# jmhb0/view_neti

Measured on AMD Instinct MI355X. Metric: TI train steps/sec (SD-1.5 512^2 bs=4 per GPU), higher is better.
Workload: dtype f16; 1 GPU; learnable_mode 0, sd15 shapes, 512x512 fp16, bs=4/GPU, grad_accum 1, full train step (VAE+16xCLIP+UNet fwd/bwd+AdamW); global_batch=4, parallelism=dp1, rccl_ranks=1, hipgraph=True

## Files before the change

### include/vneti.h

```cpp
#ifndef VNETI_H
#define VNETI_H
#include <stddef.h>
#include <stdint.h>

#ifdef __cplusplus
extern "C" {
#endif

#define VNETI_ABI_VERSION 1

int vneti_version(void);
int vneti_precision(void);
int vneti_last_error(char* buf, size_t n);

typedef struct vneti_gemm_desc {
  const void* A;
  const void* B;
  void* C;
  long long lda, ldb, ldc;
  int M, N, K;
  int batch;
  long long strideA, strideB, strideC;
  const float* bias;
  const void* rowadd;
// ... 83 lines not shown
int vneti_attn_bwd_delta(const void* dO, long long lddo, const void* O, long long ldo,
                         float* delta, int Bn, int H, int Nq, int D, void* stream);
int vneti_attn_bwd_dq(const void* Q, long long ldq, const void* K, long long ldk, const void* V,
                      long long ldv, const void* dO, long long lddo, const float* lse, float* delta,
                      const void* O, long long ldo, void* dQ, long long lddq, int Bn, int H, int Nq,
                      int Nk, int D, float scale, int causal, void* stream);
int vneti_attn_bwd_dkv(const void* Q, long long ldq, const void* K, long long ldk, const void* V,
                       long long ldv, const void* dO, long long lddo, const float* lse,
                       const float* delta, void* dK, long long lddk, void* dV, long long lddv,
                       int Bn, int H, int Nq, int Nk, int D, float scale, int causal, float* ws,
                       long long ws_floats, void* stream);
int vneti_attn_bwd_small(const void* Q, long long ldq, const void* K, long long ldk, const void* V, long long ldv,
                         const void* dO, long long lddo, const void* O, long long ldo, const float* lse, void* dQ,
                         long long lddq, void* dK, long long lddk, void* dV, long long lddv, int Bn, int H, int N, int D,
                         float scale, int causal, void* stream);
int vneti_softmax_rows_f16(void* x, long long ld, int rows, int cols, void* stream);

int vneti_add_f16(const void* a, long long lda, const void* b, long long ldb, void* out,
                  long long ldo, int rows, int cols, void* stream);
int vneti_geglu_fwd(const void* p, long long ldp, void* out, long long ldo, int rows, int C4,
                    void* stream);
int vneti_geglu_bwd(const void* dy, long long lddy, const void* p, long long ldp, void* dp,
                    long long lddp, int rows, int C4, void* stream);
int vneti_act_fwd_f16(const void* x, void* y, long long n, int act, void* stream);
int vneti_act_bwd_f16(const void* dy, const void* x, void* dx, long long n, int act, void* stream);
int vneti_timestep_embedding(const void* t, void* out, int Bn, int dim, void* stream);
int vneti_sum2x2_f16(const void* in, long long ldi, void* out, long long ldo, int Bn, int H, int W,
                     int C, void* stream);
int vneti_rng_fill_normal(void* out_f32, long long n, const void* state, unsigned stream_id,
                          void* stream);
// ... 74 lines not shown
                                  const int* slot, long long slot_stride, int accumulate, int nl, int Bn, int enc_dim,
                                  int pe_dim, void* stream);
int vneti_text_embed(const float* tok_emb, const float* pos_emb, const void* ids_i64,
                     const int* pos_obj, const float* word_obj, const int* pos_view,
                     const float* word_view, float* X, int nl, int Bn, int L, int D, void* stream);
int vneti_text_final_fwd(const float* last, const float* gamma, const float* beta, float eps,
                         const int* pos_obj, const float* bypass_obj, float alpha_obj,
                         int unconstrained_obj, const int* pos_view, const float* bypass_view,
                         float alpha_view, int unconstrained_view, float* norm_terms, void* ctx_k,
                         void* ctx_v, int nl, int Bn, int L, int D, void* stream);
int vneti_text_final_bwd(const float* last, const float* gamma, float eps, const int* pos_obj,
                         const float* bypass_obj, float alpha_obj, int unconstrained_obj,
                         float* dbypass_obj, const int* pos_view, const float* bypass_view,
                         float alpha_view, int unconstrained_view, float* dbypass_view,
                         const float* norm_terms, const void* dctx_k, const void* dctx_v, float* dX,
                         int nl, int Bn, int L, int D, void* stream);
int vneti_mapper_inputs(const void* timesteps_i64, const float* view_params, int nv, float* data,
                        int nl, int Bn, void* stream);
int vneti_cast_f32_f16(const float* x, void* y, long long n, void* stream);


int vneti_img_resample_ksize(int in_size, int out_size, int filter);
int vneti_img_resample_coeffs(int in_size, int out_size, int filter, int* bounds, int* kk, void* stream);
int vneti_img_resample_pass(const void* in, int in_w, void* out, int out_h, int out_w, const int* bounds,
                            const int* kk, int ksize, int horizontal, void* stream);
int vneti_img_crop(const void* in, int in_w, int top, int left, void* out, int h, int w, int flip, void* stream);
int vneti_img_enhance(void* img, int h, int w, int mode, float alpha, void* scratch8, void* stream);
int vneti_img_hue(void* img, int h, int w, int shift, void* stream);
int vneti_img_blur5(const void* in, void* out, float* tmp, int h, int w, const float* k5_host, void* stream);
int vneti_img_affine_nearest(const void* in, void* out, int h, int w, const int* a6_host, int fill, void* stream);
int vneti_img_to_f32_chw(const void* img, float* out, int h, int w, void* stream);
// ... 23 lines not shown
```

### view_neti_amd/csrc/attention.hip

```cpp
#include "common.h"
#include "../../include/vneti.h"

namespace {

constexpr float LOG2E = 1.4426950408889634f;
constexpr int TROW64 = 144;
constexpr int TROW32 = 80;
constexpr int DKV_QH(int D) { return D <= 64 ? 2 : 1; }

template <int D>
struct Cfg {
  static constexpr int KS = (D + 15) / 16;
  static constexpr int DPAD = KS * 16;
  static constexpr int DB = (D + 31) / 32;
  static constexpr int DCH = D / 8;
  static constexpr int ROW = DPAD * 2 + 16;
};

struct AttnArgs {
  const half_t *Q, *K, *V, *dO;
  half_t *O, *dQ, *dK, *dV;
  float* lse;
  const float* lse_in;
  const float* delta;
// ... 633 lines not shown
      for (int qd = 0; qd < 4; ++qd) {
        int d = db * 32 + 8 * qd + 4 * h2;
        if (d < D) {
          half4 k4 = {(half_t)(dk[db][4 * qd] * a.scale), (half_t)(dk[db][4 * qd + 1] * a.scale),
                      (half_t)(dk[db][4 * qd + 2] * a.scale), (half_t)(dk[db][4 * qd + 3] * a.scale)};
          half4 v4 = {(half_t)dv[db][4 * qd], (half_t)dv[db][4 * qd + 1], (half_t)dv[db][4 * qd + 2],
                      (half_t)dv[db][4 * qd + 3]};
          *reinterpret_cast<half4*>(krow + d) = k4;
          *reinterpret_cast<half4*>(vrow + d) = v4;
        }
      }
    }
  }
}

template <int D>
__global__ __launch_bounds__(256, 2) void attn_bwd_small_kernel(AttnArgs a) {
  using C = Cfg<D>;
  constexpr int NR = 96;
  constexpr int TILE = NR * C::ROW + 128;
  __shared__ __attribute__((aligned(16))) char smem[4 * TILE + 2 * NR * 4];
  char* Qs = smem;
  char* Ks = smem + TILE;
  char* Vs = smem + 2 * TILE;
  char* dOs = smem + 3 * TILE;
  float* lses = reinterpret_cast<float*>(smem + 4 * TILE);
  float* dels = lses + NR;

  const int tid = threadIdx.x, lane = tid & 63, wave = tid >> 6;
  const int l31 = lane & 31, h2 = lane >> 5;
  const int b = blockIdx.y, h = blockIdx.x;
  const int N = a.Nq;

  __amdgpu_buffer_rsrc_t rsQ = vn_make_rsrc(a.Q, (uint32_t)((long long)a.Bn * N * a.ldq * 2));
  __amdgpu_buffer_rsrc_t rsdO = vn_make_rsrc(a.dO, (uint32_t)((long long)a.Bn * N * a.lddo * 2));
// ... 4 lines not shown
  constexpr int NIT = (NR * C::DCH + 255) / 256;
  u32x4 rq[NIT], rk[NIT], rv[NIT], rd[NIT];
#pragma unroll
  for (int i = 0; i < NIT; ++i) {
    const int idx = tid + 256 * i;
    const int r = idx / C::DCH, cc = idx - r * C::DCH;
    const bool ok = idx < NR * C::DCH && r < N;
    const long long row = (long long)b * N + r;
    rq[i] = vn_buf_load16(rsQ, ok ? (uint32_t)((row * a.ldq + h * D + cc * 8) * 2) : VN_OOB);
    rk[i] = vn_buf_load16(rsK, ok ? (uint32_t)((row * a.ldk + h * D + cc * 8) * 2) : VN_OOB);
    rv[i] = vn_buf_load16(rsV, ok ? (uint32_t)((row * a.ldv + h * D + cc * 8) * 2) : VN_OOB);
    rd[i] = vn_buf_load16(rsdO, ok ? (uint32_t)((row * a.lddo + h * D + cc * 8) * 2) : VN_OOB);
  }
  float lreg = INFINITY;
  if (tid < NR && tid < N) lreg = a.lse_in[((long long)b * a.H + h) * N + tid] * LOG2E;
  zero_lds(smem, 4 * TILE);
  __syncthreads();
#pragma unroll
  for (int i = 0; i < NIT; ++i) {
    const int idx = tid + 256 * i;
    const int r = idx / C::DCH, cc = idx - r * C::DCH;
    if (idx < NR * C::DCH) {
      *reinterpret_cast<u32x4*>(Qs + r * C::ROW + cc * 16) = rq[i];
      *reinterpret_cast<u32x4*>(Ks + r * C::ROW + cc * 16) = rk[i];
      *reinterpret_cast<u32x4*>(Vs + r * C::ROW + cc * 16) = rv[i];
      *reinterpret_cast<u32x4*>(dOs + r * C::ROW + cc * 16) = rd[i];
    }
  }
  if (tid < NR) lses[tid] = lreg;
  __syncthreads();

  const float c = a.scale * LOG2E;
  const int row = wave * 32 + l31;
  const bool rok = row < N;
  if (wave < 3) {
    half8 qf[C::KS], dof[C::KS];
    float part = 0.f;
#pragma unroll
    for (int ks = 0; ks < C::KS; ++ks) {
      const int ch = ks * 2 + h2;
      qf[ks] = as_half8(*reinterpret_cast<const u32x4*>(Qs + row * C::ROW + ch * 16));
      dof[ks] = as_half8(*reinterpret_cast<const u32x4*>(dOs + row * C::ROW + ch * 16));
      const uint32_t offo = (rok && ch < C::DCH) ? (uint32_t)((((long long)b * N + row) * a.ldo + h * D + ch * 8) * 2) : VN_OOB;
      const half8 of = as_half8(vn_buf_load16(rsO, offo));
#pragma unroll
      for (int j = 0; j < 8; ++j) part += (float)dof[ks][j] * (float)of[j];
    }
    const float dlt = part + __shfl_xor(part, 32, 64);
    if (h2 == 0) dels[row] = dlt;
    const float lse2 = lses[row];
    f32x16 dq[C::DB];
#pragma unroll
    for (int i = 0; i < C::DB; ++i)
#pragma unroll
      for (int e = 0; e < 16; ++e) dq[i][e] = 0.f;
    const int nkb = a.causal ? wave + 1 : 3;
    for (int aa = 0; aa < nkb; ++aa) {
      f32x16 s, dp;
#pragma unroll
      for (int e = 0; e < 16; ++e) {
        s[e] = 0.f;
        dp[e] = 0.f;
      }
#pragma unroll
      for (int ks = 0; ks < C::KS; ++ks) {
        const int off = (aa * 32 + l31) * C::ROW + (ks * 2 + h2) * 16;
        half8 kf = as_half8(*reinterpret_cast<const u32x4*>(Ks + off));
        half8 vf = as_half8(*reinterpret_cast<const u32x4*>(Vs + off));
        s = VN_MFMA_32x32x16(kf, qf[ks], s, 0, 0, 0);
        dp = VN_MFMA_32x32x16(vf, dof[ks], dp, 0, 0, 0);
      }
      if (aa * 32 + 32 > N || (a.causal && aa == wave)) {
#pragma unroll
        for (int r = 0; r < 16; ++r) {
          const int key = aa * 32 + (r & 3) + 8 * (r >> 2) + 4 * h2;
          const bool ok = key < N && (!a.causal || key <= row);
          if (!ok) s[r] = -INFINITY;
        }
      }
#pragma unroll
      for (int r = 0; r < 16; r += 2) {
        const f32x2 t = pk_fma(f32x2{s[r], s[r + 1]}, f32x2{c, c}, f32x2{-lse2, -lse2});
        const f32x2 g = f32x2{dp[r], dp[r + 1]} - f32x2{dlt, dlt};
        const f32x2 ds = f32x2{fast_exp2(t.x), fast_exp2(t.y)} * g;
        s[r] = ds.x;
        s[r + 1] = ds.y;
      }
#pragma unroll
      for (int j = 0; j < 2; ++j) {
        half8 pf = cvt8(s, j);
#pragma unroll
        for (int db = 0; db < C::DB; ++db) {
          half8 tf = load_tr(Ks, C::ROW, db * 32, aa * 32 + 16 * j + 4 * h2, lane);
          dq[db] = VN_MFMA_32x32x16(tf, pf, dq[db], 0, 0, 0);
        }
      }
    }
    if (rok) {
      half_t* orow = a.dQ + ((long long)b * N + row) * a.lddq + h * D;
#pragma unroll
      for (int db = 0; db < C::DB; ++db)
#pragma unroll
        for (int qd = 0; qd < 4; ++qd) {
          const int d = db * 32 + 8 * qd + 4 * h2;
          if (d < D) {
            half4 v = {(half_t)(dq[db][4 * qd] * a.scale), (half_t)(dq[db][4 * qd + 1] * a.scale),
                       (half_t)(dq[db][4 * qd + 2] * a.scale), (half_t)(dq[db][4 * qd + 3] * a.scale)};
            *reinterpret_cast<half4*>(orow + d) = v;
          }
        }
    }
  }
  __syncthreads();
  if (wave < 3) {
    half8 kf[C::KS], vf[C::KS];
#pragma unroll
    for (int ks = 0; ks < C::KS; ++ks) {
      const int ch = ks * 2 + h2;
      kf[ks] = as_half8(*reinterpret_cast<const u32x4*>(Ks + row * C::ROW + ch * 16));
      vf[ks] = as_half8(*reinterpret_cast<const u32x4*>(Vs + row * C::ROW + ch * 16));
    }
    f32x16 dk[C::DB], dv[C::DB];
#pragma unroll
    for (int i = 0; i < C::DB; ++i)
#pragma unroll
      for (int e = 0; e < 16; ++e) {
        dk[i][e] = 0.f;
        dv[i][e] = 0.f;
      }
    for (int hq = a.causal ? wave : 0; hq < 3; ++hq) {
      f32x16 s, dp;
#pragma unroll
      for (int e = 0; e < 16; ++e) {
        s[e] = 0.f;
        dp[e] = 0.f;
      }
#pragma unroll
      for (int ks = 0; ks < C::KS; ++ks) {
        const int off = (hq * 32 + l31) * C::ROW + (ks * 2 + h2) * 16;
        half8 qfr = as_half8(*reinterpret_cast<const u32x4*>(Qs + off));
        half8 dofr = as_half8(*reinterpret_cast<const u32x4*>(dOs + off));
        s = VN_MFMA_32x32x16(qfr, kf[ks], s, 0, 0, 0);
        dp = VN_MFMA_32x32x16(dofr, vf[ks], dp, 0, 0, 0);
      }
#pragma unroll
      for (int qd = 0; qd < 4; ++qd) {
        f32x4 l4 = *reinterpret_cast<const f32x4*>(&lses[hq * 32 + 8 * qd + 4 * h2]);
        f32x4 d4 = *reinterpret_cast<const f32x4*>(&dels[hq * 32 + 8 * qd + 4 * h2]);
#pragma unroll
        for (int e = 0; e < 4; e += 2) {
          const int r = 4 * qd + e;
          const f32x2 t = pk_fma(f32x2{s[r], s[r + 1]}, f32x2{c, c}, -f32x2{l4[e], l4[e + 1]});
          f32x2 p = f32x2{fast_exp2(t.x), fast_exp2(t.y)};
          if (a.causal) {
// ... 2 lines not shown
            if (row > qq + 1) p.y = 0.f;
          }
          const f32x2 ds = p * (f32x2{dp[r], dp[r + 1]} - f32x2{d4[e], d4[e + 1]});
          s[r] = p.x;
          s[r + 1] = p.y;
          dp[r] = ds.x;
          dp[r + 1] = ds.y;
        }
      }
#pragma unroll
      for (int j = 0; j < 2; ++j) {
        half8 pf = cvt8(s, j);
        half8 dsf = cvt8(dp, j);
#pragma unroll
        for (int db = 0; db < C::DB; ++db) {
          half8 dot = load_tr(dOs, C::ROW, db * 32, hq * 32 + 16 * j + 4 * h2, lane);
          half8 qtf = load_tr(Qs, C::ROW, db * 32, hq * 32 + 16 * j + 4 * h2, lane);
          dv[db] = VN_MFMA_32x32x16(dot, pf, dv[db], 0, 0, 0);
          dk[db] = VN_MFMA_32x32x16(qtf, dsf, dk[db], 0, 0, 0);
        }
      }
    }
    if (rok) {
      half_t* krow = a.dK + ((long long)b * N + row) * a.lddk + h * D;
      half_t* vrow = a.dV + ((long long)b * N + row) * a.lddv + h * D;
#pragma unroll
      for (int db = 0; db < C::DB; ++db)
#pragma unroll
        for (int qd = 0; qd < 4; ++qd) {
          const int d = db * 32 + 8 * qd + 4 * h2;
          if (d < D) {
            half4 k4 = {(half_t)(dk[db][4 * qd] * a.scale), (half_t)(dk[db][4 * qd + 1] * a.scale),
                        (half_t)(dk[db][4 * qd + 2] * a.scale), (half_t)(dk[db][4 * qd + 3] * a.scale)};
            half4 v4 = {(half_t)dv[db][4 * qd], (half_t)dv[db][4 * qd + 1], (half_t)dv[db][4 * qd + 2],
                        (half_t)dv[db][4 * qd + 3]};
            *reinterpret_cast<half4*>(krow + d) = k4;
            *reinterpret_cast<half4*>(vrow + d) = v4;
          }
        }
    }
  }
}

__global__ __launch_bounds__(256) void attn_dkv_reduce_kernel(AttnArgs a) {
  const int Cc = a.H * a.D;
  const long long rows = (long long)a.Bn * a.Nk;
  const long long plane = rows * Cc;
  const unsigned gid = blockIdx.x * 256u + threadIdx.x;
  if (gid >= (unsigned)(plane / 4)) return;
  const unsigned e32 = gid * 4u;
  const unsigned row32 = e32 / (unsigned)Cc;
  const int c = (int)(e32 - row32 * (unsigned)Cc);
  const long long e = e32, row = row32;
  f32x4 k = {0.f, 0.f, 0.f, 0.f}, v = {0.f, 0.f, 0.f, 0.f};
  for (int s = 0; s < a.qsplit; ++s) {
// ... 156 lines not shown
    if (qsplit < 2) qsplit = 1;
  }
  a.qsplit = qsplit;
  a.ws = ws;
  dim3 grid(nkb * qsplit, H, Bn);
  hipStream_t st = (hipStream_t)stream;
  DISPATCH_D(attn_dkv_kernel, grid, st, a);
  if (qsplit > 1) {
    long long n4 = (long long)Bn * Nk * H * D / 4;
    VN_REQUIRE(n4 * 4 < 0x7fffffffLL, "attn_bwd_dkv: q-split reduce indexes with 32 bits");
    hipLaunchKernelGGL(attn_dkv_reduce_kernel, dim3((unsigned)cdivl(n4, 256)), dim3(256), 0, st, a);
  }
  return vneti_check_launch("attn_bwd_dkv");
}

extern "C" int vneti_attn_bwd_small(const void* Q, long long ldq, const void* K, long long ldk, const void* V, long long ldv,
                                    const void* dO, long long lddo, const void* O, long long ldo, const float* lse, void* dQ,
                                    long long lddq, void* dK, long long lddk, void* dV, long long lddv, int Bn, int H, int N,
                                    int D, float scale, int causal, void* stream) {
  VN_REQUIRE(Q && K && V && dO && O && lse && dQ && dK && dV, "attn_bwd_small: null pointer");
  VN_REQUIRE(Bn > 0 && H > 0 && N > 0, "attn_bwd_small: bad shape B=%d H=%d N=%d", Bn, H, N);
  if (N > 96 || D != 64) return VNETI_EUNSUP;
  VN_REQUIRE(ldq % 8 == 0 && ldk % 8 == 0 && ldv % 8 == 0 && lddo % 8 == 0 && ldo % 8 == 0 && lddq % 4 == 0 && lddk % 4 == 0 &&
                 lddv % 4 == 0, "attn_bwd_small: bad strides");
  AttnArgs a;
  memset(&a, 0, sizeof(a));
  a.Q = (const half_t*)Q;
  a.K = (const half_t*)K;
  a.V = (const half_t*)V;
  a.dO = (const half_t*)dO;
// ... 24 lines not shown
```

### view_neti_amd/csrc/text.hip

```cpp
#include "common.h"
#include "../../include/vneti.h"

namespace {

constexpr int MAXH = 192;

struct MapperParams {
  int w0, b0, g1, be1, w3, b3, g2, be2, wo, bo;
  int E, hd, OD, D;
};

__device__ __forceinline__ float leaky(float x) { return x > 0.f ? x : 0.01f * x; }

constexpr int MT = 1024;

__device__ __forceinline__ float group16_sum(float s) {
  s += vn_row_ror<8>(s);
  s += vn_row_ror<4>(s);
  s += vn_row_ror<2>(s);
  s += vn_row_ror<1>(s);
  return s;
}

__device__ __forceinline__ float block_sum(float v, float* red) {
// ... 631 lines not shown
#pragma unroll
          for (int j = 0; j < 8; ++j) x[i][j] += f * bv[i][j];
      }
      changed = true;
    }
  }
  if (changed) row_stats(x, D, eps, mean, rstd);
  row_ln_store(x, D, lane, mean, rstd, gamma, beta, ctx_v + row * D);
}

__global__ __launch_bounds__(256) void text_final_bwd_kernel(const float* __restrict__ last,
                                                             const float* __restrict__ gamma, float eps,
                                                             BypassArgs obj, BypassArgs view,
                                                             const half_t* __restrict__ dctx_k,
                                                             const half_t* __restrict__ dctx_v,
                                                             float* __restrict__ dX, int nl, int Bn, int L, int D) {
  const long long row = (long long)blockIdx.x * 4 + (threadIdx.x >> 6);
  const int lane = threadIdx.x & 63;
  if (row >= (long long)nl * Bn * L) return;
  const int pos = (int)(row % L);
  const int b = (int)((row / L) % Bn);
  const int l = (int)(row / ((long long)L * Bn));
  float x[TMAX][8], g1[TMAX][8];
  row_load(last + row * D, D, lane, x);
  row_ln_bwd(x, dctx_k + row * D, D, lane, eps, gamma, g1);
  const bool is_obj = obj.pos && obj.pos[b] == pos;
  const bool is_view = view.pos && view.pos[b] == pos;
  float g2[TMAX][8];
  if (!is_obj && !is_view) {
    row_ln_bwd(x, dctx_v + row * D, D, lane, eps, gamma, g2);
  } else {
// ... 17 lines not shown
#pragma unroll
      for (int j = 0; j < 8; ++j) {
        g2[i][j] = unc ? 0.f : g[i][j] + a.alpha * ug * x[i][j] / nx;
        if (c * 8 < D) dbp[c * 8 + j] = f * (g[i][j] - bv[i][j] / nb * ug);
      }
    }
  }
#pragma unroll
  for (int i = 0; i < TMAX; ++i) {
    int c = lane + 64 * i;
    if (c * 8 < D) {
      f32x4 o0 = {g1[i][0] + g2[i][0], g1[i][1] + g2[i][1], g1[i][2] + g2[i][2], g1[i][3] + g2[i][3]};
      f32x4 o1 = {g1[i][4] + g2[i][4], g1[i][5] + g2[i][5], g1[i][6] + g2[i][6], g1[i][7] + g2[i][7]};
      *reinterpret_cast<f32x4*>(dX + row * D + c * 8) = o0;
      *reinterpret_cast<f32x4*>(dX + row * D + c * 8 + 4) = o1;
    }
  }
}

__global__ void mapper_inputs_kernel(const long long* __restrict__ t, const float* __restrict__ view_params, int nv,
                                     float* __restrict__ data, int nl, int Bn) {
  int gid = blockIdx.x * blockDim.x + threadIdx.x;
  int nf = 2 + nv;
  if (gid >= nl * Bn * nf) return;
  int f = gid % nf;
  int r = gid / nf;
  int b = r % Bn, l = r / Bn;
  float v;
  if (f == 0) v = (float)t[b] / 1000.f * 2.f - 1.f;
  else if (f == 1) v = (float)l / (float)nl * 2.f - 1.f;
// ... 185 lines not shown
               uv ? norm_terms + (long long)nl * Bn : nullptr};
  if (uo || uv)
    hipLaunchKernelGGL(text_norm_terms_kernel, dim3(nl * Bn), dim3(256), 0, ST, last, o, uo ? 1 : 0, norm_terms, nl,
                       Bn, L, D);
  long long rows = (long long)nl * Bn * L;
  hipLaunchKernelGGL(text_final_fwd_kernel, dim3((unsigned)cdivl(rows, 4)), dim3(256), 0, ST, last, gamma, beta, eps, o,
                     v, (half_t*)ctx_k, (half_t*)ctx_v, nl, Bn, L, D);
  return vneti_check_launch("text_final_fwd");
}

extern "C" int vneti_text_final_bwd(const float* last, const float* gamma, float eps, const int* pos_obj,
                                    const float* bypass_obj, float alpha_obj, int unconstrained_obj,
                                    float* dbypass_obj, const int* pos_view, const float* bypass_view,
                                    float alpha_view, int unconstrained_view, float* dbypass_view,
                                    const float* norm_terms, const void* dctx_k, const void* dctx_v, float* dX,
                                    int nl, int Bn, int L, int D, void* stream) {
  VN_REQUIRE(last && gamma && dctx_k && dctx_v && dX && D % 8 == 0 && D <= 8 * 64 * TMAX, "text_final_bwd: bad arguments");
  VN_REQUIRE(!(pos_obj && bypass_obj && !dbypass_obj) && !(pos_view && bypass_view && !dbypass_view),
             "text_final_bwd: missing bypass gradient buffer");
  const bool uo = unconstrained_obj && pos_obj && bypass_obj, uv = unconstrained_view && pos_view && bypass_view;
  VN_REQUIRE(!(uo || uv) || norm_terms, "text_final_bwd: unconstrained bypass needs the forward's norm_terms");
  BypassArgs o{pos_obj && bypass_obj ? pos_obj : nullptr, bypass_obj, dbypass_obj, alpha_obj, uo ? norm_terms : nullptr};
  BypassArgs v{pos_view && bypass_view ? pos_view : nullptr, bypass_view, dbypass_view, alpha_view,
               uv ? norm_terms + (long long)nl * Bn : nullptr};
  long long rows = (long long)nl * Bn * L;
  hipLaunchKernelGGL(text_final_bwd_kernel, dim3((unsigned)cdivl(rows, 4)), dim3(256), 0, ST, last, gamma, eps, o, v,
                     (const half_t*)dctx_k, (const half_t*)dctx_v, dX, nl, Bn, L, D);
  return vneti_check_launch("text_final_bwd");
}

extern "C" int vneti_mapper_inputs(const void* timesteps, const float* view_params, int nv, float* data, int nl,
                                   int Bn, void* stream) {
  VN_REQUIRE(timesteps && data && nl > 0 && Bn > 0 && nv >= 0 && (nv == 0 || view_params), "mapper_inputs: bad arguments");
  int n = nl * Bn * (2 + nv);
  hipLaunchKernelGGL(mapper_inputs_kernel, dim3(cdiv(n, 256)), dim3(256), 0, ST, (const long long*)timesteps,
                     view_params, nv, data, nl, Bn);
  return vneti_check_launch("mapper_inputs");
}

extern "C" int vneti_cast_f32_f16(const float* x, void* y, long long n, void* stream) {
  VN_REQUIRE(x && y && n > 0 && n % 8 == 0, "cast_f32_f16: n must be a positive multiple of 8");
  hipLaunchKernelGGL(cast_f32_f16_kernel, dim3((unsigned)cdivl(n / 8, 256)), dim3(256), 0, ST, x, (half_t*)y, n / 8);
// ... 3 lines not shown
```

### view_neti_amd/engine/text.py

```python
from __future__ import annotations

from functools import partial
from typing import Dict, Optional

import torch

from .. import ops
from .. import sd_config as sc
from .schedule import Schedule, rup


class MapperState:

    def __init__(self, params: torch.Tensor, w_enc: Optional[torch.Tensor], norm_scale: Optional[float], alpha: float,
                 hidden: int = 64, enc_dim: int = 64, unconstrained: bool = False, nested_dropout_prob: float = 0.0,
                 slot: Optional[torch.Tensor] = None, slot_stride: int = 0, legacy_w_pe: Optional[torch.Tensor] = None,
                 output_bypass: bool = True, slots: Optional[torch.Tensor] = None):
        self.output_bypass = output_bypass
        self.legacy_w_pe = legacy_w_pe
        self.pe_dim = 2 * legacy_w_pe.shape[0] if legacy_w_pe is not None else 0
        self.params = params
        self.w_enc = w_enc
        self.norm_scale = norm_scale
        self.alpha = alpha
# ... 208 lines not shown
        act = ops.ACT_QUICK_GELU if cfg.act == "quick_gelu" else ops.ACT_GELU
        for i in range(cfg.num_layers):
            p = f"text_model.encoder.layers.{i}."
            r = dict(x_in=x, act=act)
            n1, r["ln1"] = self._ln(x, p + "layer_norm1", w)
            wqkv = torch.cat([w[p + "self_attn.q_proj.weight"], w[p + "self_attn.k_proj.weight"],
                              w[p + "self_attn.v_proj.weight"]], 0)
            bqkv = torch.cat([w[p + "self_attn.q_proj.bias"], w[p + "self_attn.k_proj.bias"],
                              w[p + "self_attn.v_proj.bias"]], 0)
            r["wqkv"], r_bqkv = self._w16(wqkv), self._w32(bqkv)
            qkv = self._buf((Rt, 3 * D))
            f.append(partial(ops.gemm, n1, r["wqkv"], qkv, bias=r_bqkv))
            q, k, v = qkv[:, :D], qkv[:, D:2 * D], qkv[:, 2 * D:]
            o = self._buf((Rt, D))
            lse = self._buf((R, H, L), torch.float32)
            f.append(partial(ops.attn_fwd, q, k, v, o, lse, R, H, L, L, hd, hd ** -0.5, True))
            r["wo"], bo_ = self._w16(w[p + "self_attn.out_proj.weight"]), self._w32(w[p + "self_attn.out_proj.bias"])
            x_mid = self._buf((Rt, D), torch.float32)
            f.append(partial(ops.gemm, o, r["wo"], x_mid, bias=bo_, resid=x))
            n2, r["ln2"] = self._ln(x_mid, p + "layer_norm2", w)
            r["w1"], b1 = self._w16(w[p + "mlp.fc1.weight"]), self._w32(w[p + "mlp.fc1.bias"])
            r["w2"], b2 = self._w16(w[p + "mlp.fc2.weight"]), self._w32(w[p + "mlp.fc2.bias"])
            f1 = self._buf((Rt, F))
            a1 = self._buf((Rt, F))
            f.append(partial(ops.gemm, n2, r["w1"], f1, bias=b1, out2=a1, act2=act))
            x_out = self._buf((Rt, D), torch.float32)
            f.append(partial(ops.gemm, a1, r["w2"], x_out, bias=b2, resid=x_mid))
            r.update(qkv=qkv, o=o, lse=lse, x_mid=x_mid, f1=f1)
            if self.need_backward:
                tr = lambda t: self._w16(t.t())
                r["w2d"], r["w1d"] = tr(w[p + "mlp.fc2.weight"]), tr(w[p + "mlp.fc1.weight"])
# ... 9 lines not shown
                                            self.mo.alpha, self.pos_view, byp_v,
                                            self.mv.alpha if self.mv else 0.0, self.ctx_k, self.ctx_v, nl, B, L, D,
                                            self.mo.unconstrained, bool(self.mv and self.mv.unconstrained),
                                            self.norm_terms))

    def _build_backward(self):
        cfg = self.cfg
        B, L, D, nl, R, Rt = self.B, self.L, cfg.hidden_size, self.nl, self.R, self.Rt
        H = cfg.num_heads
        hd = D // H
        F = cfg.intermediate_size
        bw = self.bwd
        dx = self._buf((Rt, D), torch.float32)
        byp_o = self.bo["byp"] if self.mo.output_bypass else None
        byp_v = self.bv["byp"] if (self.bv and self.mv.output_bypass) else None
        bw.append(lambda: ops.text_final_bwd(self.last, self.fln_g, cfg.eps, self.pos_obj, byp_o,
                                             self.mo.alpha, self.bo["dbyp"] if byp_o is not None else None, self.pos_view,
                                             byp_v, self.mv.alpha if self.mv else 0.0,
                                             self.bv["dbyp"] if byp_v is not None else None, self.dctx_k, self.dctx_v, dx, nl, B,
                                             L, D, self.mo.unconstrained, bool(self.mv and self.mv.unconstrained),
                                             self.norm_terms))
        g16 = self._buf((Rt, D))
        dxm = self._buf((Rt, D), torch.float32)
        bw.append(partial(ops.cast_f32_f16, dx, g16))
        for r in reversed(self.layers):
            qkv = r["qkv"]
            q, k, v = qkv[:, :D], qkv[:, D:2 * D], qkv[:, 2 * D:]
            df1 = self._tmp("cB", Rt, F)
            bw.append(partial(ops.gemm, g16, r["w2d"], df1, gate=r["f1"], gate_act=r["act"]))
            dn2 = self._tmp("cC", Rt, D)
            bw.append(partial(ops.gemm, df1, r["w1d"], dn2))
            bw.append(partial(self._ln_bwd, r["ln2"], dn2, dxm, dx, g16))
            do = self._tmp("cD", Rt, D)
            bw.append(partial(ops.gemm, g16, r["wod"], do))
            delta = self._tmp("cdelta", R * H, L, torch.float32)
            dqkv = self._tmp("cE", Rt, 3 * D)
            dq, dk, dv = dqkv[:, :D], dqkv[:, D:2 * D], dqkv[:, 2 * D:]
            sc_ = hd ** -0.5
            if ops.attn_bwd_small_ok(L, hd):
# ... 24 lines not shown
```

### view_neti_amd/ops.py

```python
from __future__ import annotations

import ctypes as C

import torch

from . import lib as _l

ACT_NONE, ACT_SILU, ACT_QUICK_GELU, ACT_GELU = 0, 1, 2, 3


def stream() -> int:
    return torch.cuda.current_stream().cuda_stream


def _p(t):
    return None if t is None else t.data_ptr()


def _ld(t):
    if t is None:
        return 0
    assert t.stride(-1) == 1, "last dim must be contiguous"
    return t.stride(-2) if t.dim() >= 2 else t.shape[-1]

# ... 149 lines not shown
    ws = workspace if workspace is not None else _default_ws
    _l.call("attn_bwd_dkv", _p(Q), _ld(Q), _p(K), _ld(K), _p(V), _ld(V), _p(dO), _ld(dO), _p(lse), _p(delta),
            _p(dK), _ld(dK), _p(dV), _ld(dV), Bn, H, Nq, Nk, D, scale, 1 if causal else 0, _p(ws),
            ws.numel() if ws is not None else 0, stream())


def attn_bwd_small_ok(N, D):
    return N <= 96 and D == 64


def attn_bwd_small(Q, K, V, dO, O, lse, dQ, dK, dV, Bn, H, N, D, scale, causal):
    _l.call("attn_bwd_small", _p(Q), _ld(Q), _p(K), _ld(K), _p(V), _ld(V), _p(dO), _ld(dO), _p(O), _ld(O), _p(lse),
            _p(dQ), _ld(dQ), _p(dK), _ld(dK), _p(dV), _ld(dV), Bn, H, N, D, scale, 1 if causal else 0, stream())


def softmax_rows(x, rows, cols):
    _l.call("softmax_rows_f16", _p(x), _ld(x), rows, cols, stream())


def add(a, b, out):
    rows, cols = out.shape
    _l.call("add_f16", _p(a), _ld(a), _p(b), _ld(b), _p(out), _ld(out), rows, cols, stream())


def geglu_fwd(p, out):
    rows, c4 = out.shape
    _l.call("geglu_fwd", _p(p), _ld(p), _p(out), _ld(out), rows, c4, stream())


def geglu_bwd(dy, p, dp):
# ... 185 lines not shown

def text_embed(tok_emb, pos_emb, ids, pos_obj, word_obj, pos_view, word_view, X, nl, Bn, L, D):
    _l.call("text_embed", _p(tok_emb), _p(pos_emb), _p(ids), _p(pos_obj), _p(word_obj), _p(pos_view), _p(word_view),
            _p(X), nl, Bn, L, D, stream())


def text_final_fwd(last, gamma, beta, eps, pos_obj, byp_obj, alpha_obj, pos_view, byp_view, alpha_view, ctx_k, ctx_v,
                   nl, Bn, L, D, unconstrained_obj=False, unconstrained_view=False, norm_terms=None):
    _l.call("text_final_fwd", _p(last), _p(gamma), _p(beta), eps, _p(pos_obj), _p(byp_obj), alpha_obj,
            1 if unconstrained_obj else 0, _p(pos_view), _p(byp_view), alpha_view, 1 if unconstrained_view else 0,
            _p(norm_terms), _p(ctx_k), _p(ctx_v), nl, Bn, L, D, stream())


def text_final_bwd(last, gamma, eps, pos_obj, byp_obj, alpha_obj, dbyp_obj, pos_view, byp_view, alpha_view, dbyp_view,
                   dctx_k, dctx_v, dX, nl, Bn, L, D, unconstrained_obj=False, unconstrained_view=False,
                   norm_terms=None):
    _l.call("text_final_bwd", _p(last), _p(gamma), eps, _p(pos_obj), _p(byp_obj), alpha_obj,
            1 if unconstrained_obj else 0, _p(dbyp_obj), _p(pos_view), _p(byp_view), alpha_view,
            1 if unconstrained_view else 0, _p(dbyp_view), _p(norm_terms), _p(dctx_k), _p(dctx_v), _p(dX), nl, Bn, L,
            D, stream())


def cast_f32_f16(x, y):
    _l.call("cast_f32_f16", _p(x), _p(y), x.numel(), stream())


def mapper_inputs(timesteps, view_params, data, nl, Bn):
    nv = 0 if view_params is None else view_params.shape[1]
    _l.call("mapper_inputs", _p(timesteps), _p(view_params), nv, _p(data), nl, Bn, stream())


def gemm_select_split(M, N, K, batch, tile_hint, workspace_bytes):
    return _l.query("gemm_select_split", M, N, K, batch, tile_hint, workspace_bytes)


# ... 77 lines not shown
```

### view_neti_amd/roofline.py

```python
from __future__ import annotations

import torch

from . import ops

import os as _os

_CSRC = _os.path.join(_os.path.dirname(_os.path.abspath(__file__)), "csrc")
MFMA_PEAK_TFLOPS = 2500.0
HBM_PEAK_TBS = 8.0
PF, TB = MFMA_PEAK_TFLOPS, HBM_PEAK_TBS


def kernel_tree_sha() -> str:
    import hashlib
    import os
    here = _CSRC
    files = sorted(os.path.join(here, f) for f in os.listdir(here) if f.endswith((".hip", ".h")))
    files.append(os.path.join(os.path.dirname(os.path.dirname(here)), "include", "vneti.h"))
    h = hashlib.sha256()
    for f in files:
        h.update(os.path.basename(f).encode())
        h.update(open(f, "rb").read())
    return h.hexdigest()[:16]
# ... 13 lines not shown
    if kw.get("geglu") == 1:
        extra -= M * N
    nbytes = a_bytes + N * K * 2 * batch + M * c_cols * out.element_size() * batch + extra
    flops = 2.0 * M * N * K * batch
    return M, N, K, batch, flops, nbytes, flops / (MFMA_PEAK_TFLOPS * 1e12), nbytes / (HBM_PEAK_TBS * 1e12)



def cost(f):
    fn, a, kw = getattr(f, "func", None), getattr(f, "args", ()), getattr(f, "keywords", {}) or {}
    if fn is ops.gemm:
        M, N, K, batch, flops, nbytes, t_mfma, t_hbm = gemm_cost(f)
        if t_hbm > t_mfma:
            return ("gemm, below the ridge (short-K linears: HBM-bound)", 0, nbytes)
        return ("gemm / implicit-GEMM conv (MFMA-bound)", flops, 0)
    if fn in (ops.attn_fwd, ops.attn_bwd_dq, ops.attn_bwd_dkv):
        i = {ops.attn_fwd: 5, ops.attn_bwd_dq: 7, ops.attn_bwd_dkv: 8}[fn]
        Bn, H, Nq, Nk, D = a[i:i + 5]
        causal = a[i + 6]
        mm = {ops.attn_fwd: 2, ops.attn_bwd_dq: 3, ops.attn_bwd_dkv: 4}[fn]
        name = {ops.attn_fwd: "attention fwd", ops.attn_bwd_dq: "attention bwd dQ", ops.attn_bwd_dkv: "attention bwd dK/dV"}[fn]
        scores = Bn * H * Nq * Nk * (0.5 if causal else 1.0)
        ks, db = -(-D // 16), -(-D // 32)
        mfma_c = {ops.attn_fwd: ks + 2 * db, ops.attn_bwd_dq: 2 * ks + 2 * db, ops.attn_bwd_dkv: 2 * ks + 4 * db}[fn] * 32 / 1024.0
        valu_c = {ops.attn_fwd: 2.8, ops.attn_bwd_dq: 4.0, ops.attn_bwd_dkv: 4.0}[fn] * 2 / 64.0 + (2 * 5 / 3) / 64.0
        cob = scores * (mfma_c + valu_c) / (1024 * 2.4e9)
        return (name, mm * 2.0 * scores * D, 0, cob)
    if fn is ops.attn_bwd_small:
        Bn, H, N, D = a[9:13]
        return ("attention bwd (short sequences, one launch)", 7 * 2.0 * Bn * H * N * N * D * (0.5 if a[14] else 1.0), 0)
# ... 89 lines not shown
```

Measured before the change: 38.70 steps/s.

## Add single-tile CLIP attention forward, swizzle small-attn LDS, fuse f16 grad cast

Adds a dedicated forward attention kernel for short sequences (N<=96, head dim 64), used by the CLIP text encoder. It keeps the whole K/V tile in LDS and computes each block in one pass. The small backward kernel now uses an unpadded XOR-swizzled LDS layout instead of a padded one, which drops the LDS zeroing and raises the occupancy hint from 2 to 3 blocks. The f16 copy of the text-final gradient is now written inside text_final_bwd, removing a separate cast launch. These target launch and latency overhead in the text path, which is a small share of a full SD-1.5 train step, so the effect on the step is likely minor.

```diff
diff --git a/include/vneti.h b/include/vneti.h
--- a/include/vneti.h
+++ b/include/vneti.h
@@ -121,6 +121,9 @@
                          const void* dO, long long lddo, const void* O, long long ldo, const float* lse, void* dQ,
                          long long lddq, void* dK, long long lddk, void* dV, long long lddv, int Bn, int H, int N, int D,
                          float scale, int causal, void* stream);
+int vneti_attn_fwd_small(const void* Q, long long ldq, const void* K, long long ldk, const void* V, long long ldv,
+                         void* O, long long ldo, float* lse, int Bn, int H, int N, int D, float scale, int causal,
+                         void* stream);
 int vneti_softmax_rows_f16(void* x, long long ld, int rows, int cols, void* stream);
 
 int vneti_add_f16(const void* a, long long lda, const void* b, long long ldb, void* out,
@@ -225,7 +228,7 @@
                          float* dbypass_obj, const int* pos_view, const float* bypass_view,
                          float alpha_view, int unconstrained_view, float* dbypass_view,
                          const float* norm_terms, const void* dctx_k, const void* dctx_v, float* dX,
-                         int nl, int Bn, int L, int D, void* stream);
+                         void* dX16, int nl, int Bn, int L, int D, void* stream);
 int vneti_mapper_inputs(const void* timesteps_i64, const float* view_params, int nv, float* data,
                         int nl, int Bn, void* stream);
 int vneti_cast_f32_f16(const float* x, void* y, long long n, void* stream);
diff --git a/view_neti_amd/csrc/attention.hip b/view_neti_amd/csrc/attention.hip
--- a/view_neti_amd/csrc/attention.hip
+++ b/view_neti_amd/csrc/attention.hip
@@ -671,11 +671,29 @@
   }
 }
 
+constexpr int SMALL_NR = 96;
+constexpr int SMALL_ROW = 128;
+__device__ __forceinline__ int small_off(int r, int ch) {
+  return r * SMALL_ROW + ((ch ^ (((r >> 2) & 3) | ((r & 2) << 1))) << 4);
+}
+__device__ __forceinline__ half8 load_tr_small(const char* tile, int d0, int n0, int lane) {
+  const int i = lane & 15;
+  const int r = n0 + (i >> 2);
+  const int hb = (d0 + 16 * ((lane >> 4) & 1) + 4 * (i & 3)) * 2;
+  typedef __attribute__((address_space(3))) vn_short4* lds_ptr;
+  vn_short4 lo = __builtin_amdgcn_ds_read_tr16_b64_v4i16((lds_ptr)(tile + small_off(r, hb >> 4) + (hb & 15)));
+  vn_short4 hi = __builtin_amdgcn_ds_read_tr16_b64_v4i16((lds_ptr)(tile + small_off(r + 8, hb >> 4) + (hb & 15)));
+  half4 l4 = __builtin_bit_cast(half4, lo), h4 = __builtin_bit_cast(half4, hi);
+  half8 v = {l4[0], l4[1], l4[2], l4[3], h4[0], h4[1], h4[2], h4[3]};
+  return v;
+}
+
 template <int D>
-__global__ __launch_bounds__(256, 2) void attn_bwd_small_kernel(AttnArgs a) {
+__global__ __launch_bounds__(256, 3) void attn_bwd_small_kernel(AttnArgs a) {
   using C = Cfg<D>;
-  constexpr int NR = 96;
-  constexpr int TILE = NR * C::ROW + 128;
+  static_assert(C::DPAD == D && D * 2 == SMALL_ROW, "the unpadded swizzled tile is laid out for d = 64");
+  constexpr int NR = SMALL_NR;
+  constexpr int TILE = NR * SMALL_ROW;
   __shared__ __attribute__((aligned(16))) char smem[4 * TILE + 2 * NR * 4];
   char* Qs = smem;
   char* Ks = smem + TILE;
@@ -710,17 +728,15 @@
   }
   float lreg = INFINITY;
   if (tid < NR && tid < N) lreg = a.lse_in[((long long)b * a.H + h) * N + tid] * LOG2E;
-  zero_lds(smem, 4 * TILE);
-  __syncthreads();
 #pragma unroll
   for (int i = 0; i < NIT; ++i) {
     const int idx = tid + 256 * i;
     const int r = idx / C::DCH, cc = idx - r * C::DCH;
     if (idx < NR * C::DCH) {
-      *reinterpret_cast<u32x4*>(Qs + r * C::ROW + cc * 16) = rq[i];
-      *reinterpret_cast<u32x4*>(Ks + r * C::ROW + cc * 16) = rk[i];
-      *reinterpret_cast<u32x4*>(Vs + r * C::ROW + cc * 16) = rv[i];
-      *reinterpret_cast<u32x4*>(dOs + r * C::ROW + cc * 16) = rd[i];
+      *reinterpret_cast<u32x4*>(Qs + small_off(r, cc)) = rq[i];
+      *reinterpret_cast<u32x4*>(Ks + small_off(r, cc)) = rk[i];
+      *reinterpret_cast<u32x4*>(Vs + small_off(r, cc)) = rv[i];
+      *reinterpret_cast<u32x4*>(dOs + small_off(r, cc)) = rd[i];
     }
   }
   if (tid < NR) lses[tid] = lreg;
@@ -735,8 +751,8 @@
 #pragma unroll
     for (int ks = 0; ks < C::KS; ++ks) {
       const int ch = ks * 2 + h2;
-      qf[ks] = as_half8(*reinterpret_cast<const u32x4*>(Qs + row * C::ROW + ch * 16));
-      dof[ks] = as_half8(*reinterpret_cast<const u32x4*>(dOs + row * C::ROW + ch * 16));
+      qf[ks] = as_half8(*reinterpret_cast<const u32x4*>(Qs + small_off(row, ch)));
+      dof[ks] = as_half8(*reinterpret_cast<const u32x4*>(dOs + small_off(row, ch)));
       const uint32_t offo = (rok && ch < C::DCH) ? (uint32_t)((((long long)b * N + row) * a.ldo + h * D + ch * 8) * 2) : VN_OOB;
       const half8 of = as_half8(vn_buf_load16(rsO, offo));
 #pragma unroll
@@ -760,7 +776,7 @@
       }
 #pragma unroll
       for (int ks = 0; ks < C::KS; ++ks) {
-        const int off = (aa * 32 + l31) * C::ROW + (ks * 2 + h2) * 16;
+        const int off = small_off(aa * 32 + l31, ks * 2 + h2);
         half8 kf = as_half8(*reinterpret_cast<const u32x4*>(Ks + off));
         half8 vf = as_half8(*reinterpret_cast<const u32x4*>(Vs + off));
         s = VN_MFMA_32x32x16(kf, qf[ks], s, 0, 0, 0);
@@ -787,7 +803,7 @@
         half8 pf = cvt8(s, j);
 #pragma unroll
         for (int db = 0; db < C::DB; ++db) {
-          half8 tf = load_tr(Ks, C::ROW, db * 32, aa * 32 + 16 * j + 4 * h2, lane);
+          half8 tf = load_tr_small(Ks, db * 32, aa * 32 + 16 * j + 4 * h2, lane);
           dq[db] = VN_MFMA_32x32x16(tf, pf, dq[db], 0, 0, 0);
         }
       }
@@ -813,8 +829,8 @@
 #pragma unroll
     for (int ks = 0; ks < C::KS; ++ks) {
       const int ch = ks * 2 + h2;
-      kf[ks] = as_half8(*reinterpret_cast<const u32x4*>(Ks + row * C::ROW + ch * 16));
-      vf[ks] = as_half8(*reinterpret_cast<const u32x4*>(Vs + row * C::ROW + ch * 16));
+      kf[ks] = as_half8(*reinterpret_cast<const u32x4*>(Ks + small_off(row, ch)));
+      vf[ks] = as_half8(*reinterpret_cast<const u32x4*>(Vs + small_off(row, ch)));
     }
     f32x16 dk[C::DB], dv[C::DB];
 #pragma unroll
@@ -833,7 +849,7 @@
       }
 #pragma unroll
       for (int ks = 0; ks < C::KS; ++ks) {
-        const int off = (hq * 32 + l31) * C::ROW + (ks * 2 + h2) * 16;
+        const int off = small_off(hq * 32 + l31, ks * 2 + h2);
         half8 qfr = as_half8(*reinterpret_cast<const u32x4*>(Qs + off));
         half8 dofr = as_half8(*reinterpret_cast<const u32x4*>(dOs + off));
         s = VN_MFMA_32x32x16(qfr, kf[ks], s, 0, 0, 0);
@@ -866,8 +882,8 @@
         half8 dsf = cvt8(dp, j);
 #pragma unroll
         for (int db = 0; db < C::DB; ++db) {
-          half8 dot = load_tr(dOs, C::ROW, db * 32, hq * 32 + 16 * j + 4 * h2, lane);
-          half8 qtf = load_tr(Qs, C::ROW, db * 32, hq * 32 + 16 * j + 4 * h2, lane);
+          half8 dot = load_tr_small(dOs, db * 32, hq * 32 + 16 * j + 4 * h2, lane);
+          half8 qtf = load_tr_small(Qs, db * 32, hq * 32 + 16 * j + 4 * h2, lane);
           dv[db] = VN_MFMA_32x32x16(dot, pf, dv[db], 0, 0, 0);
           dk[db] = VN_MFMA_32x32x16(qtf, dsf, dk[db], 0, 0, 0);
         }
@@ -891,6 +907,155 @@
           }
         }
     }
+  }
+}
+
+__global__ __launch_bounds__(192, 3) void attn_fwd_small_kernel(AttnArgs a) {
+  constexpr int D = 64;
+  using C = Cfg<D>;
+  constexpr int NR = SMALL_NR;
+  constexpr int TILE = NR * SMALL_ROW;
+  __shared__ __attribute__((aligned(16))) char smem[2 * TILE];
+  char* Ks = smem;
+  char* Vs = smem + TILE;
+
+  const int tid = threadIdx.x, lane = tid & 63, wave = tid >> 6;
+  const int l31 = lane & 31, h2 = lane >> 5;
+  const int b = blockIdx.y, h = blockIdx.x;
+  const int N = a.Nq;
+  const int q = wave * 32 + l31;
+  const bool qok = q < N;
+
+  __amdgpu_buffer_rsrc_t rsQ = vn_make_rsrc(a.Q, (uint32_t)((long long)a.Bn * N * a.ldq * 2));
+  __amdgpu_buffer_rsrc_t rsK = vn_make_rsrc(a.K, (uint32_t)((long long)a.Bn * N * a.ldk * 2));
+  __amdgpu_buffer_rsrc_t rsV = vn_make_rsrc(a.V, (uint32_t)((long long)a.Bn * N * a.ldv * 2));
+
+  constexpr int NIT = NR * C::DCH / 192;
+  static_assert(NIT * 192 == NR * C::DCH, "the tile is a whole number of 16-byte chunks per thread");
+  u32x4 rk[NIT], rv[NIT];
+#pragma unroll
+  for (int i = 0; i < NIT; ++i) {
+    const int idx = tid + 192 * i;
+    const int r = idx / C::DCH, cc = idx - r * C::DCH;
+    const long long row = (long long)b * N + r;
+    rk[i] = vn_buf_load16(rsK, r < N ? (uint32_t)((row * a.ldk + h * D + cc * 8) * 2) : VN_OOB);
+    rv[i] = vn_buf_load16(rsV, r < N ? (uint32_t)((row * a.ldv + h * D + cc * 8) * 2) : VN_OOB);
+  }
+  half8 qf[C::KS];
+#pragma unroll
+  for (int ks = 0; ks < C::KS; ++ks) {
+    const int ch = ks * 2 + h2;
+    qf[ks] = as_half8(vn_buf_load16(rsQ, qok ? (uint32_t)((((long long)b * N + q) * a.ldq + h * D + ch * 8) * 2) : VN_OOB));
+  }
+#pragma unroll
+  for (int i = 0; i < NIT; ++i) {
+    const int idx = tid + 192 * i;
+    const int r = idx / C::DCH, cc = idx - r * C::DCH;
+    *reinterpret_cast<u32x4*>(Ks + small_off(r, cc)) = rk[i];
+    *reinterpret_cast<u32x4*>(Vs + small_off(r, cc)) = rv[i];
+  }
+
+  f32x16 o[C::DB];
+  float m = -INFINITY, l = 0.f;
+#pragma unroll
+  for (int i = 0; i < C::DB; ++i)
+#pragma unroll
+    for (int e = 0; e < 16; ++e) o[i][e] = 0.f;
+  const float c = a.scale * LOG2E;
+
+  int nkt = cdiv_dev(N, 64);
+  if (a.causal) nkt = min(nkt, (N - 1) / 64 + 1);
+  __syncthreads();
+  for (int kt = 0; kt < nkt; ++kt) {
+    const int key0 = kt * 64;
+    if (a.causal && key0 > wave * 32 + 31) continue;
+    f32x16 s[2];
+#pragma unroll
+    for (int aa = 0; aa < 2; ++aa)
+#pragma unroll
+      for (int e = 0; e < 16; ++e) s[aa][e] = 0.f;
+#pragma unroll
+    for (int aa = 0; aa < 2; ++aa) {
+      if (key0 + aa * 32 < NR) {
+#pragma unroll
+        for (int ks = 0; ks < C::KS; ++ks) {
+          half8 kf = as_half8(*reinterpret_cast<const u32x4*>(Ks + small_off(key0 + aa * 32 + l31, ks * 2 + h2)));
+          s[aa] = VN_MFMA_32x32x16(kf, qf[ks], s[aa], 0, 0, 0);
+        }
+      }
+    }
+    if ((key0 + 64 > N) || a.causal) {
+#pragma unroll
+      for (int aa = 0; aa < 2; ++aa)
+#pragma unroll
+        for (int r = 0; r < 16; ++r) {
+          int key = key0 + aa * 32 + (r & 3) + 8 * (r >> 2) + 4 * h2;
+          bool ok = key < N && (!a.causal || key <= q);
+          if (!ok) s[aa][r] = -INFINITY;
+        }
+    }
+    float mx = -INFINITY;
+#pragma unroll
+    for (int aa = 0; aa < 2; ++aa)
+#pragma unroll
+      for (int r = 0; r < 16; ++r) mx = fmaxf(mx, s[aa][r]);
+    mx = fmaxf(mx, __shfl_xor(mx, 32, 64));
+    if (!__all((mx - m) * c <= RESCALE_THR_LOG2)) {
+      const float m_new = fmaxf(m, mx);
+      const float m_use = (m_new == -INFINITY) ? 0.f : m_new;
+      const float alpha = fast_exp2((m - m_use) * c);
+      l *= alpha;
+      m = m_use;
+#pragma unroll
+      for (int i = 0; i < C::DB; ++i)
+#pragma unroll
+        for (int e = 0; e < 16; ++e) o[i][e] *= alpha;
+    }
+    const float mc = m * c;
+    float psum = 0.f;
+#pragma unroll
+    for (int aa = 0; aa < 2; ++aa) {
+#pragma unroll
+      for (int r = 0; r < 16; r += 2) {
+        const f32x2 t = pk_fma(f32x2{s[aa][r], s[aa][r + 1]}, f32x2{c, c}, f32x2{-mc, -mc});
+        const float p0 = fast_exp2(t.x), p1 = fast_exp2(t.y);
+        s[aa][r] = p0;
+        s[aa][r + 1] = p1;
+        psum += p0 + p1;
+      }
+    }
+    l += psum;
+#pragma unroll
+    for (int aa = 0; aa < 2; ++aa) {
+      if (key0 + aa * 32 < NR) {
+#pragma unroll
+        for (int j = 0; j < 2; ++j) {
+          half8 pf = cvt8(s[aa], j);
+#pragma unroll
+          for (int db = 0; db < C::DB; ++db) {
+            half8 vf = load_tr_small(Vs, db * 32, key0 + aa * 32 + 16 * j + 4 * h2, lane);
+            o[db] = VN_MFMA_32x32x16(vf, pf, o[db], 0, 0, 0);
+          }
+        }
+      }
+    }
+  }
+
+  const float lt = l + __shfl_xor(l, 32, 64);
+  const float inv = (lt > 0.f) ? 1.f / lt : 0.f;
+  if (qok) {
+    half_t* orow = a.O + ((long long)b * N + q) * a.ldo + h * D;
+#pragma unroll
+    for (int db = 0; db < C::DB; ++db) {
+#pragma unroll
+      for (int qd = 0; qd < 4; ++qd) {
+        int d = db * 32 + 8 * qd + 4 * h2;
+        half4 v = {(half_t)(o[db][4 * qd] * inv), (half_t)(o[db][4 * qd + 1] * inv), (half_t)(o[db][4 * qd + 2] * inv),
+                   (half_t)(o[db][4 * qd + 3] * inv)};
+        *reinterpret_cast<half4*>(orow + d) = v;
+      }
+    }
+    if (h2 == 0 && a.lse) a.lse[((long long)b * a.H + h) * N + q] = m * a.scale + logf(lt);
   }
 }
 
@@ -1077,6 +1242,36 @@
   return vneti_check_launch("attn_bwd_dkv");
 }
 
+extern "C" int vneti_attn_fwd_small(const void* Q, long long ldq, const void* K, long long ldk, const void* V, long long ldv,
+                                    void* O, long long ldo, float* lse, int Bn, int H, int N, int D, float scale, int causal,
+                                    void* stream) {
+  VN_REQUIRE(Q && K && V && O, "attn_fwd_small: null pointer");
+  VN_REQUIRE(Bn > 0 && H > 0 && N > 0, "attn_fwd_small: bad shape B=%d H=%d N=%d", Bn, H, N);
+  if (N > 96 || D != 64) return VNETI_EUNSUP;
+  VN_REQUIRE(ldq % 8 == 0 && ldk % 8 == 0 && ldv % 8 == 0 && ldo % 4 == 0, "attn_fwd_small: bad strides");
+  VN_REQUIRE(Bn <= 65535, "attn_fwd_small: more than 65535 sequences");
+  AttnArgs a;
+  memset(&a, 0, sizeof(a));
+  a.Q = (const half_t*)Q;
+  a.K = (const half_t*)K;
+  a.V = (const half_t*)V;
+  a.O = (half_t*)O;
+  a.lse = lse;
+  a.ldq = ldq;
+  a.ldk = ldk;
+  a.ldv = ldv;
+  a.ldo = ldo;
+  a.Bn = Bn;
+  a.H = H;
+  a.Nq = N;
+  a.Nk = N;
+  a.D = D;
+  a.scale = scale;
+  a.causal = causal;
+  hipLaunchKernelGGL(attn_fwd_small_kernel, dim3(H, Bn), dim3(192), 0, (hipStream_t)stream, a);
+  return vneti_check_launch("attn_fwd_small");
+}
+
 extern "C" int vneti_attn_bwd_small(const void* Q, long long ldq, const void* K, long long ldk, const void* V, long long ldv,
                                     const void* dO, long long lddo, const void* O, long long ldo, const float* lse, void* dQ,
                                     long long lddq, void* dK, long long lddk, void* dV, long long lddv, int Bn, int H, int N,
diff --git a/view_neti_amd/csrc/text.hip b/view_neti_amd/csrc/text.hip
--- a/view_neti_amd/csrc/text.hip
+++ b/view_neti_amd/csrc/text.hip
@@ -669,7 +669,8 @@
                                                              BypassArgs obj, BypassArgs view,
                                                              const half_t* __restrict__ dctx_k,
                                                              const half_t* __restrict__ dctx_v,
-                                                             float* __restrict__ dX, int nl, int Bn, int L, int D) {
+                                                             float* __restrict__ dX, half_t* __restrict__ dX16, int nl,
+                                                             int Bn, int L, int D) {
   const long long row = (long long)blockIdx.x * 4 + (threadIdx.x >> 6);
   const int lane = threadIdx.x & 63;
   if (row >= (long long)nl * Bn * L) return;
@@ -717,6 +718,11 @@
       f32x4 o1 = {g1[i][4] + g2[i][4], g1[i][5] + g2[i][5], g1[i][6] + g2[i][6], g1[i][7] + g2[i][7]};
       *reinterpret_cast<f32x4*>(dX + row * D + c * 8) = o0;
       *reinterpret_cast<f32x4*>(dX + row * D + c * 8 + 4) = o1;
+      if (dX16) {
+        half8 h = {(half_t)o0[0], (half_t)o0[1], (half_t)o0[2], (half_t)o0[3],
+                   (half_t)o1[0], (half_t)o1[1], (half_t)o1[2], (half_t)o1[3]};
+        *reinterpret_cast<half8*>(dX16 + row * D + c * 8) = h;
+      }
     }
   }
 }
@@ -932,7 +938,7 @@
                                     float* dbypass_obj, const int* pos_view, const float* bypass_view,
                                     float alpha_view, int unconstrained_view, float* dbypass_view,
                                     const float* norm_terms, const void* dctx_k, const void* dctx_v, float* dX,
-                                    int nl, int Bn, int L, int D, void* stream) {
+                                    void* dX16, int nl, int Bn, int L, int D, void* stream) {
   VN_REQUIRE(last && gamma && dctx_k && dctx_v && dX && D % 8 == 0 && D <= 8 * 64 * TMAX, "text_final_bwd: bad arguments");
   VN_REQUIRE(!(pos_obj && bypass_obj && !dbypass_obj) && !(pos_view && bypass_view && !dbypass_view),
              "text_final_bwd: missing bypass gradient buffer");
@@ -943,7 +949,7 @@
                uv ? norm_terms + (long long)nl * Bn : nullptr};
   long long rows = (long long)nl * Bn * L;
   hipLaunchKernelGGL(text_final_bwd_kernel, dim3((unsigned)cdivl(rows, 4)), dim3(256), 0, ST, last, gamma, eps, o, v,
-                     (const half_t*)dctx_k, (const half_t*)dctx_v, dX, nl, Bn, L, D);
+                     (const half_t*)dctx_k, (const half_t*)dctx_v, dX, (half_t*)dX16, nl, Bn, L, D);
   return vneti_check_launch("text_final_bwd");
 }
 
diff --git a/view_neti_amd/engine/text.py b/view_neti_amd/engine/text.py
--- a/view_neti_amd/engine/text.py
+++ b/view_neti_amd/engine/text.py
@@ -246,7 +246,10 @@
             q, k, v = qkv[:, :D], qkv[:, D:2 * D], qkv[:, 2 * D:]
             o = self._buf((Rt, D))
             lse = self._buf((R, H, L), torch.float32)
-            f.append(partial(ops.attn_fwd, q, k, v, o, lse, R, H, L, L, hd, hd ** -0.5, True))
+            if ops.attn_fwd_small_ok(L, hd):
+                f.append(partial(ops.attn_fwd_small, q, k, v, o, lse, R, H, L, hd, hd ** -0.5, True))
+            else:
+                f.append(partial(ops.attn_fwd, q, k, v, o, lse, R, H, L, L, hd, hd ** -0.5, True))
             r["wo"], bo_ = self._w16(w[p + "self_attn.out_proj.weight"]), self._w32(w[p + "self_attn.out_proj.bias"])
             x_mid = self._buf((Rt, D), torch.float32)
             f.append(partial(ops.gemm, o, r["wo"], x_mid, bias=bo_, resid=x))
@@ -286,15 +289,14 @@
         dx = self._buf((Rt, D), torch.float32)
         byp_o = self.bo["byp"] if self.mo.output_bypass else None
         byp_v = self.bv["byp"] if (self.bv and self.mv.output_bypass) else None
+        g16 = self._buf((Rt, D))
         bw.append(lambda: ops.text_final_bwd(self.last, self.fln_g, cfg.eps, self.pos_obj, byp_o,
                                              self.mo.alpha, self.bo["dbyp"] if byp_o is not None else None, self.pos_view,
                                              byp_v, self.mv.alpha if self.mv else 0.0,
                                              self.bv["dbyp"] if byp_v is not None else None, self.dctx_k, self.dctx_v, dx, nl, B,
                                              L, D, self.mo.unconstrained, bool(self.mv and self.mv.unconstrained),
-                                             self.norm_terms))
-        g16 = self._buf((Rt, D))
+                                             self.norm_terms, f16_copy=g16))
         dxm = self._buf((Rt, D), torch.float32)
-        bw.append(partial(ops.cast_f32_f16, dx, g16))
         for r in reversed(self.layers):
             qkv = r["qkv"]
             q, k, v = qkv[:, :D], qkv[:, D:2 * D], qkv[:, 2 * D:]
diff --git a/view_neti_amd/ops.py b/view_neti_amd/ops.py
--- a/view_neti_amd/ops.py
+++ b/view_neti_amd/ops.py
@@ -187,6 +187,15 @@
             _p(dQ), _ld(dQ), _p(dK), _ld(dK), _p(dV), _ld(dV), Bn, H, N, D, scale, 1 if causal else 0, stream())
 
 
+def attn_fwd_small_ok(N, D):
+    return N <= 96 and D == 64
+
+
+def attn_fwd_small(Q, K, V, O, lse, Bn, H, N, D, scale, causal):
+    _l.call("attn_fwd_small", _p(Q), _ld(Q), _p(K), _ld(K), _p(V), _ld(V), _p(O), _ld(O), _p(lse), Bn, H, N, D, scale,
+            1 if causal else 0, stream())
+
+
 def softmax_rows(x, rows, cols):
     _l.call("softmax_rows_f16", _p(x), _ld(x), rows, cols, stream())
 
@@ -402,11 +411,11 @@
 
 def text_final_bwd(last, gamma, eps, pos_obj, byp_obj, alpha_obj, dbyp_obj, pos_view, byp_view, alpha_view, dbyp_view,
                    dctx_k, dctx_v, dX, nl, Bn, L, D, unconstrained_obj=False, unconstrained_view=False,
-                   norm_terms=None):
+                   norm_terms=None, f16_copy=None):
     _l.call("text_final_bwd", _p(last), _p(gamma), eps, _p(pos_obj), _p(byp_obj), alpha_obj,
             1 if unconstrained_obj else 0, _p(dbyp_obj), _p(pos_view), _p(byp_view), alpha_view,
-            1 if unconstrained_view else 0, _p(dbyp_view), _p(norm_terms), _p(dctx_k), _p(dctx_v), _p(dX), nl, Bn, L,
-            D, stream())
+            1 if unconstrained_view else 0, _p(dbyp_view), _p(norm_terms), _p(dctx_k), _p(dctx_v), _p(dX), _p(f16_copy),
+            nl, Bn, L, D, stream())
 
 
 def cast_f32_f16(x, y):
diff --git a/view_neti_amd/roofline.py b/view_neti_amd/roofline.py
--- a/view_neti_amd/roofline.py
+++ b/view_neti_amd/roofline.py
@@ -51,6 +51,8 @@
         if t_hbm > t_mfma:
             return ("gemm, below the ridge (short-K linears: HBM-bound)", 0, nbytes)
         return ("gemm / implicit-GEMM conv (MFMA-bound)", flops, 0)
+    if fn is ops.attn_fwd_small:
+        fn, a = ops.attn_fwd, (*a[:7], a[7], *a[7:])
     if fn in (ops.attn_fwd, ops.attn_bwd_dq, ops.attn_bwd_dkv):
         i = {ops.attn_fwd: 5, ops.attn_bwd_dq: 7, ops.attn_bwd_dkv: 8}[fn]
         Bn, H, Nq, Nk, D = a[i:i + 5]
```

Result: no change. 38.87 steps/s, median of 6 (+0.4%).
